# sIncerass/MVLPT

Measured on AMD Instinct MI355X. Metric: prompt-tuning images/sec (fwd+bwd), ViT-B/16 bs=256, 1/2/4/8 MI355X, higher is better.
Workload: dtype fp16; 1 GPU; BASELINE configs[1]: MVLPT coop head, ViT-B/16, 100 classes (caltech101 token table), n_ctx=16 n_vpt=0, text L=77, class token middle; text_positions_evaluated=77, step_pipelining=True, grad_precision=split_grad, layernorm_folding=both towers, residual_stream=packed fp16 + byte (image tower without prompts / backward), cu_partition=none (towers share every compute unit), per_gpu_batch=256, global_batch=256, parallelism=dp1, text_tower=replicated per GPU

## Files before the change

include/mvlpt_hip.h:

```cpp
#ifndef MVLPT_HIP_H
#define MVLPT_HIP_H
#include <stdint.h>
#ifdef __cplusplus
extern "C" {
#endif

typedef void* mvlpt_stream_t;

enum { MVLPT_DT_F32 = 0, MVLPT_DT_F16 = 1, MVLPT_DT_BF16 = 2 };
enum { MVLPT_LABEL_INT64 = 0, MVLPT_LABEL_PROB_F32 = 1 };
enum { MVLPT_ERR_ARG = -1, MVLPT_ERR_HIP = -2, MVLPT_ERR_STATE = -3, MVLPT_ERR_UNSUPPORTED = -4 };

typedef struct MvlptArch {
  int image_resolution, patch_size, vision_width, vision_layers, vision_heads;
  int context_length, text_width, text_layers, text_heads;
  int embed_dim;
  int compute_dtype;
} MvlptArch;

enum { MVLPT_PREC_FAST = 0, MVLPT_PREC_SPLIT_GRAD = 1, MVLPT_PREC_SPLIT_ALL = 2 };

int mvlpt_create(const MvlptArch* arch, void** handle);
int mvlpt_set_precision(void* handle, int mode);
int mvlpt_set_ln_fold(void* handle, int mode, int min_rows);
// ... 61 lines not shown
int mvlpt_op_attention32_bwd(int dtype, const void* qkv, const void* out, const void* dout, const float* lse, float* delta,
                             void* dqkv, int N, int L, int H, int causal, mvlpt_stream_t stream);
int mvlpt_op_pack_weight_mixed(int dtype, const float* w32, int rows, int cols, int transposed, void* out, int* w8_exp,
                               mvlpt_stream_t stream);
int mvlpt_op_gemm_mixed(int dtype, int epi, const void* A, const void* Bt, int ldb, int w8_exp, int M, int N, int K, const float* bias,
                        const void* aux, const float* resid, void* out, void* out2, mvlpt_stream_t stream);
int mvlpt_op_cast_mixed(int dtype, const float* in, void* out, int64_t rows, int d, mvlpt_stream_t stream);
int mvlpt_op_fold_vectors(int dtype, const void* W16, int ld, const float* gamma, const float* beta, const float* b, float* colsum,
                          float* bias2, int N, int K, mvlpt_stream_t stream);
int mvlpt_op_gemm_ln_producer(int dtype, const void* A, int a_split, const void* Bt, int ldb, int w8_exp, int M, int N, int K,
                              const float* bias, const float* resid, const float* gamma, int x16_split, float* out32, void* x16,
                              float* part, int ntp, int* nt, mvlpt_stream_t stream);
int mvlpt_op_gemm_folded(int dtype, int epi, const void* A16, int a_split, const void* Bt, int ldb, int w8_exp, int M, int N, int K,
                         const float* colsum, const float* bias2, const float* part, int ntp, int nt, void* out, void* out2,
                         mvlpt_stream_t stream);
int mvlpt_op_fold_weight(const void* W16, int ld, const float* gamma, void* Wg16, int ldg, float* colsum, int N, int K,
                         mvlpt_stream_t stream);
int mvlpt_op_respk_pack(const float* x, void* hi, uint8_t* lo, float* part, int ntp, int rows, int d, mvlpt_stream_t stream);
int mvlpt_op_assemble_packed(const float* patch_emb, const float* cls, const float* pos, const float* ln_g, const float* ln_b, void* hi,
                             uint8_t* lo, float* part, int ntp, int batch, int grid2, int d, mvlpt_stream_t stream);
int mvlpt_op_respk_unpack(const void* hi, const uint8_t* lo, int row_mul, float* out, int rows, int d, mvlpt_stream_t stream);
int mvlpt_op_gemm_residp(const void* A, const void* Bt, int ldb, int M, int N, int K, const float* bias, const void* hi_in,
                         const uint8_t* lo_in, void* hi_out, uint8_t* lo_out, float* part, int ntp, int* nt, mvlpt_stream_t stream);
int mvlpt_op_layernorm_fwd_mixed(int out_dtype, const float* x, const float* gamma, const float* beta, void* y, int rows, int d,
                                 mvlpt_stream_t stream);
int mvlpt_op_layernorm_bwd_mixed(int dtype, const void* dy, const float* x, const float* gamma, const float* resid, float* out32,
                                 void* out16, int rows, int d, mvlpt_stream_t stream);
int mvlpt_op_attention32_fwd_mixed(int dtype, const void* qkv, void* out, float* lse, int N, int L, int H, int causal, int q_rows,
                                   mvlpt_stream_t stream);
int mvlpt_op_attention32_bwd_mixed(int dtype, const void* qkv, const void* out, const void* dout, const float* lse, float* delta,
                                   void* dqkv, int N, int L, int H, int causal, mvlpt_stream_t stream);
int mvlpt_op_layernorm_fwd(int out_dtype, const float* x, const float* gamma, const float* beta, void* y, int rows, int d,
                           mvlpt_stream_t stream);
int mvlpt_op_layernorm_bwd(int dtype, const void* dy, const float* x, const float* gamma, const float* resid, float* out32,
                           void* out16, int rows, int d, mvlpt_stream_t stream);
int mvlpt_op_attention_fwd(int dtype, const void* qkv, void* out, float* lse, int N, int L, int H, int causal,
                           mvlpt_stream_t stream);
int mvlpt_op_attention_bwd(int dtype, const void* qkv, const void* out, const void* dout, const float* lse, float* delta,
                           void* dqkv, int N, int L, int H, int causal, mvlpt_stream_t stream);
int mvlpt_op_cast(int dtype, const float* in, void* out, int64_t n, mvlpt_stream_t stream);
int mvlpt_op_assemble_prompts_grouped(const float* prefix, const float* suffix, const float* ctx, int n_ctx, const int32_t* layout,
                                      const float* pos, float* x, int G, int C, int L, int d, mvlpt_stream_t stream);
int mvlpt_op_gather_ctx_grad_grouped(const float* dx, const int32_t* ctx_pos, int G, int C, int L, int d, int n_ctx, float* dctx,
                                     mvlpt_stream_t stream);
int mvlpt_op_assemble_prompts_ranged(const float* prefix, const float* suffix, const float* ctx, int n_ctx, const int32_t* layout,
                                     const float* pos, float* x, const int32_t* class_lo, const int32_t* class_hi, int G, int C, int L,
                                     int d, mvlpt_stream_t stream);
int mvlpt_op_gather_ctx_grad_ranged(const float* dx, const int32_t* ctx_pos, const int32_t* class_lo, const int32_t* class_hi, int G, int C,
                                    int L, int d, int n_ctx, float* dctx, mvlpt_stream_t stream);

int mvlpt_op_sgemm_bt(const float* A, const float* Bt, float* C, int M, int N, int K, const float* alpha_dev, mvlpt_stream_t stream);
int mvlpt_op_grad_scale(const float* v, int64_t n, float target, float* scale_dev, mvlpt_stream_t stream);
int mvlpt_op_reduce_prompt_rows(int dtype, float* dx32, void* dx16, int B, int L, int d, int row0, int n, float* out,
                                const float* scale_dev, int zero_after, int split16, const float* vmask, mvlpt_stream_t stream);
// ... 42 lines not shown
```

mvlpt_amd/_lib.py:

```python
from __future__ import annotations

import ctypes as C
import os

import torch

_HERE = os.path.dirname(os.path.abspath(__file__))
LIB_PATH = os.environ.get("MVLPT_HIP_LIB") or os.path.join(_HERE, "libmvlpt_hip.so")

DT_F32, DT_F16, DT_BF16 = 0, 1, 2
LABEL_INT64, LABEL_PROB_F32 = 0, 1
EPI_STORE16, EPI_GELU, EPI_RESID32, EPI_GELUBWD, EPI_STORE32, EPI_GELU_SPLIT, EPI_GELUBWD_SPLIT, EPI_STORE_SPLIT = 0, 1, 2, 3, 4, 5, 6, 7
GEMM_BT_128x128_R2, GEMM_BT_128x128_R4, GEMM_BT_256x128_R3, GEMM_BT_256x256_R2, GEMM_PHASED, GEMM_PC, GEMM_PCP = 1, 2, 3, 4, 5, 6, 7
PREC_FAST, PREC_SPLIT_GRAD, PREC_SPLIT_ALL = 0, 1, 2


class MvlptArch(C.Structure):
    _fields_ = [(n, C.c_int) for n in (
        "image_resolution", "patch_size", "vision_width", "vision_layers", "vision_heads",
        "context_length", "text_width", "text_layers", "text_heads", "embed_dim", "compute_dtype")]


class MvlptKernelStat(C.Structure):
    _fields_ = [("name", C.c_char * 32), ("launches", C.c_int64), ("ms", C.c_double),
# ... 53 lines not shown
    "mvlpt_op_gemm_ln_producer": (_i, [_i, _vp, _i, _vp, _i, _i, _i, _i, _i, _vp, _vp, _vp, _i, _vp, _vp, _vp, _i, C.POINTER(C.c_int), _vp]),
    "mvlpt_op_gemm_folded": (_i, [_i, _i, _vp, _i, _vp, _i, _i, _i, _i, _i, _vp, _vp, _vp, _i, _i, _vp, _vp, _vp]),
    "mvlpt_op_fold_weight": (_i, [_vp, _i, _vp, _vp, _i, _vp, _i, _i, _vp]),
    "mvlpt_op_respk_pack": (_i, [_vp, _vp, _vp, _vp, _i, _i, _i, _vp]),
    "mvlpt_op_assemble_packed": (_i, [_vp, _vp, _vp, _vp, _vp, _vp, _vp, _vp, _i, _i, _i, _i, _vp]),
    "mvlpt_op_respk_unpack": (_i, [_vp, _vp, _i, _vp, _i, _i, _vp]),
    "mvlpt_op_gemm_residp": (_i, [_vp, _vp, _i, _i, _i, _i, _vp, _vp, _vp, _vp, _vp, _vp, _i, C.POINTER(C.c_int), _vp]),
    "mvlpt_op_layernorm_fwd_mixed": (_i, [_i, _vp, _vp, _vp, _vp, _i, _i, _vp]),
    "mvlpt_op_layernorm_bwd_mixed": (_i, [_i, _vp, _vp, _vp, _vp, _vp, _vp, _i, _i, _vp]),
    "mvlpt_op_attention32_fwd_mixed": (_i, [_i, _vp, _vp, _vp, _i, _i, _i, _i, _i, _vp]),
    "mvlpt_op_attention32_bwd_mixed": (_i, [_i, _vp, _vp, _vp, _vp, _vp, _vp, _i, _i, _i, _i, _vp]),
    "mvlpt_op_layernorm_fwd": (_i, [_i, _vp, _vp, _vp, _vp, _i, _i, _vp]),
    "mvlpt_op_layernorm_bwd": (_i, [_i, _vp, _vp, _vp, _vp, _vp, _vp, _i, _i, _vp]),
    "mvlpt_op_attention_fwd": (_i, [_i, _vp, _vp, _vp, _i, _i, _i, _i, _vp]),
    "mvlpt_op_attention_bwd": (_i, [_i, _vp, _vp, _vp, _vp, _vp, _vp, _i, _i, _i, _i, _vp]),
    "mvlpt_op_cast": (_i, [_i, _vp, _vp, C.c_int64, _vp]),
    "mvlpt_op_assemble_prompts_grouped": (_i, [_vp, _vp, _vp, _i, _vp, _vp, _vp, _i, _i, _i, _i, _vp]),
    "mvlpt_op_gather_ctx_grad_grouped": (_i, [_vp, _vp, _i, _i, _i, _i, _i, _vp, _vp]),
    "mvlpt_op_assemble_prompts_ranged": (_i, [_vp, _vp, _vp, _i, _vp, _vp, _vp, _vp, _vp, _i, _i, _i, _i, _vp]),
    "mvlpt_op_gather_ctx_grad_ranged": (_i, [_vp, _vp, _vp, _vp, _i, _i, _i, _i, _i, _vp, _vp]),
    "mvlpt_op_sgemm_bt": (_i, [_vp, _vp, _vp, _i, _i, _i, _vp, _vp]),
    "mvlpt_op_grad_scale": (_i, [_vp, C.c_int64, _f, _vp, _vp]),
    "mvlpt_op_reduce_prompt_rows": (_i, [_i, _vp, _vp, _i, _i, _i, _i, _i, _vp, _vp, _i, _i, _vp, _vp]),
    "mvlpt_op_gather_ctx_grad": (_i, [_vp, _vp, _i, _i, _i, _i, _i, _vp, _vp, _vp]),
    "mvlpt_op_attention_bwd_cls": (_i, [_i, _vp, _vp, _vp, _vp, _vp, _i, _i, _i, _vp]),
    "mvlpt_op_copy_rows": (_i, [_vp, _vp, _vp, _i, _i, _i, _vp]),
    "mvlpt_op_overwrite_rows": (_i, [_vp, _i, _vp, _i, _i, _i, _vp, _vp]),
    "mvlpt_op_assemble_tokens": (_i, [_vp, _vp, _vp, _vp, _vp, _vp, _i, _vp, _vp, _i, _i, _i, _vp]),
    "mvlpt_op_assemble_prompts": (_i, [_vp, _vp, _vp, _i, _i, _vp, _vp, _vp, _vp, _vp, _vp, _i, _i, _i, _vp]),
    "mvlpt_preprocess": (_i, [_vp, _vp, C.c_int64, C.POINTER(MvlptImageDesc), _i, _i, _i, C.POINTER(_f), C.POINTER(_f), _vp, _i, _vp, _vp]),
# ... 30 lines not shown
```

mvlpt_amd/csrc/attention.hip:

```cpp
#include <hip/hip_ext.h>
#include "attn_common.h"

namespace mvlpt {

constexpr int ATT_MAX_NKT = 38;
int attn_max_len() { return ATT_MAX_NKT * 16; }

template <typename T, int NKT, bool CAUSAL>
__global__ __launch_bounds__(256) void attn_fwd_kernel(AttnArgs a) {
  extern __shared__ __attribute__((aligned(16))) char smem[];
  using v8 = typename Vec<T>::v8;
  using v4 = typename Vec<T>::v4;
  constexpr int LP = NKT * 16;
  constexpr int BLK = NKT < 16 ? NKT : 16;
  constexpr bool PRELOAD = NKT <= 16;
  char* sK = smem;
  char* sV = smem + LP * 128;
  const int L = a.L, H = a.H, d = H * 64;
  const int n = blockIdx.x / H, h = blockIdx.x % H;
  const size_t ld = (size_t)3 * d;
  const T* base = (const T*)a.qkv + (size_t)n * L * ld + h * 64;
  const int lane = threadIdx.x & 63, wave = __builtin_amdgcn_readfirstlane(threadIdx.x >> 6);
  const int fr = lane & 15, fg = lane >> 4;
  const int nqt = a.q_rows > 0 ? ((a.q_rows < L ? a.q_rows : L) + 15) >> 4 : (L + 15) >> 4;
// ... 465 lines not shown
        *(v4*)(gp + d + dt * 16) = wv;
      }
    }
  };
  if constexpr (PRELOAD) {
#pragma unroll
    for (int ki = 0; ki < MAXK; ++ki) {
      if (wave + 4 * ki >= nkt_all) break;
      process(wave + 4 * ki, pre[ki]);
    }
  } else {
    for (int kt = wave; kt < nkt_all; kt += 4) process(kt, load_kv(kt));
  }
}

template <typename T>
__device__ __forceinline__ float cls_dot16(const float* g16, const typename Vec<T>::v8& a0, const typename Vec<T>::v8& a1) {
  float s = 0.f;
#pragma unroll
  for (int e = 0; e < 8; ++e) { s = fmaf(g16[e], to_f32<T>(a0[e]), s); s = fmaf(g16[e + 8], to_f32<T>(a1[e]), s); }
  s += __shfl_xor(s, 1, 64); s += __shfl_xor(s, 2, 64);
  return s;
}
template <typename T>
__global__ __launch_bounds__(256) void attn_bwd_cls_kernel(const T* __restrict__ qkv, const T* __restrict__ o_cls,
                                                           const T* __restrict__ do_cls, const float* __restrict__ lse,
                                                           T* __restrict__ dqkv, int N, int L, int H) {
  using v8 = typename Vec<T>::v8;
  __shared__ float sq[64], sdo[64], red[4][64];
  const int n = blockIdx.x / H, h = blockIdx.x % H, d = H * 64, tid = threadIdx.x;
// ... 163 lines not shown
```

mvlpt_amd/csrc/engine.hip:

```cpp
#include <hip/hip_runtime.h>

#include <cmath>
#include <cstdio>
#include <algorithm>
#include <array>
#include <map>
#include <cstring>
#include <mutex>
#include <string>
#include <vector>

#include "../../include/mvlpt_hip.h"
#include "kernels.h"

using namespace mvlpt;


namespace {
struct StreamPart { hipStream_t s; int cus; };
std::mutex g_part_mu;
std::vector<StreamPart> g_parts;
int device_cus() {
  static int cus = 0;
  if (!cus) {
// ... 102 lines not shown
  int vpt_mask_layers = 0, vpt_mask_B = 0, vpt_mask_n = 0, vpt_mask_d = 0;
  const float* v_mask = nullptr;
  bool lo8 = true;
  std::string err;
  TowerW vis, txt;
  void* conv_w = nullptr; int Kp = 0; float* cls_emb = nullptr; float* vpos = nullptr; LNp ln_pre, ln_post;
  float *vproj = nullptr, *vproj_t = nullptr;
  float* tpos = nullptr; LNp ln_final; float *tproj = nullptr, *tproj_t = nullptr;
  std::vector<void*> owned;
  DevBuf vis_ws, txt_ws, head_ws, ce_ws, tmp, pp_ws;
  TowerState vs, ts;
  int vB = 0, v_nvpt = 0, v_ndeep = 0; float* cls32 = nullptr; float* dcls32 = nullptr;
  float* xc32 = nullptr; void *ac16 = nullptr, *hc16 = nullptr, *gc16 = nullptr;
  bool v_cls_last = false; float *xcm32 = nullptr, *xco32 = nullptr, *dxc32 = nullptr, *dhc32 = nullptr;
  void *uc16 = nullptr, *duc16 = nullptr, *dxc16 = nullptr, *dOc16 = nullptr;
  int tC = 0, tL = 0, t_nctx = 0, t_per_class = 0; int32_t* eot_rows = nullptr; int32_t* ctx_pos = nullptr;
  int t_groups = 0, t_gC = 0;
  bool t_ranged = false; const int32_t *t_rlo = nullptr, *t_rstart = nullptr;
  std::vector<int32_t> t_range_host, h_range_host;
  bool t_eot_last = false; float *txc32 = nullptr, *txm32 = nullptr, *txo32 = nullptr, *tdxc32 = nullptr, *tdhc32 = nullptr;
  void *tac16 = nullptr, *thc16 = nullptr, *tgc16 = nullptr, *tuc16 = nullptr, *tduc16 = nullptr, *tdxc16 = nullptr, *tdOc16 = nullptr;
  float* eot32 = nullptr; float* deot32 = nullptr;
  int hB = 0, hC = 0; float h_scale = 0.f; const int32_t *h_lo = nullptr, *h_hi = nullptr;
  bool h_grouped = false;
  bool h_ranged = false; int hS = 0; const int32_t *h_rlo = nullptr, *h_rstart = nullptr, *h_rgrp = nullptr;
  float *imn = nullptr, *txn = nullptr, *inorm = nullptr, *tnorm = nullptr;
  unsigned long long* dbg_ck = nullptr; int dbg_ck_n = 0; bool dbg_ck_on = false;
  bool prof_on = false, prof_all = false; std::vector<ProfRec> prof; std::vector<hipEvent_t> ev_pool; size_t ev_used = 0;
};

// ... 633 lines not shown
  Engine* E = (Engine*)h;
  if (!E || !image || !feat_out || B <= 0) return fail(E, MVLPT_ERR_ARG, "image_fwd: null/invalid argument");
  if (int rc = mvlpt_frozen_ready(h)) return rc;
  if ((n_vpt > 0) != (vpt != nullptr)) return fail(E, MVLPT_ERR_ARG, "image_fwd: vpt pointer and n_vpt disagree");
  if ((n_deep > 0) != (vpt_deep != nullptr) || (n_deep > 0 && n_vpt <= 0)) return fail(E, MVLPT_ERR_ARG, "image_fwd: deep prompts need vpt");
  hipStream_t s = (hipStream_t)stream;
  const MvlptArch& A = E->arch;
  const int G = A.image_resolution / A.patch_size, G2 = G * G, dv = A.vision_width, e = A.embed_dim;
  const int Lv = 1 + n_vpt + G2;
  if (Lv > attn_max_len()) return fail(E, MVLPT_ERR_UNSUPPORTED, "image_fwd: sequence length > 256 not supported yet");
  const bool save = save_for_bwd != 0;
  const bool exact = E->prec_mode == MVLPT_PREC_SPLIT_ALL || (E->prec_mode == MVLPT_PREC_SPLIT_GRAD && save);
  const size_t X = exact ? 2 : 1;
  const size_t npatch = (size_t)B * G2;
  size_t need = tower_bytes(E->vis, B, Lv, save, exact) + align256(npatch * E->Kp * 2) + align256(npatch * dv * 4) +
                7 * align256((size_t)B * dv * 4) + 4 * align256((size_t)B * dv * 2 * X) + 3 * align256((size_t)B * dv * 8 * X) + 4096;
  E->vs.valid = false;
  HIPCHK(E, E->vis_ws.reserve(need));
  Bump bp; bp.base = (char*)E->vis_ws.p; bp.cap = E->vis_ws.cap;
  void* patches = bp.take_bytes(npatch * E->Kp * 2);
  float* pe = bp.take<float>(npatch * dv);
  E->cls32 = bp.take<float>((size_t)B * dv);
  E->dcls32 = bp.take<float>((size_t)B * dv);
  E->xc32 = bp.take<float>((size_t)B * dv);
  E->ac16 = bp.take_bytes((size_t)B * dv * 2 * X); E->hc16 = bp.take_bytes((size_t)B * dv * 2 * X);
  E->gc16 = bp.take_bytes((size_t)B * dv * 4 * 2 * X);
  E->xcm32 = bp.take<float>((size_t)B * dv); E->xco32 = bp.take<float>((size_t)B * dv);
  E->dxc32 = bp.take<float>((size_t)B * dv); E->dhc32 = bp.take<float>((size_t)B * dv);
  E->dxc16 = bp.take_bytes((size_t)B * dv * 2 * X); E->dOc16 = bp.take_bytes((size_t)B * dv * 2 * X);
  E->uc16 = bp.take_bytes((size_t)B * dv * 4 * 2); E->duc16 = bp.take_bytes((size_t)B * dv * 4 * 2 * X);
  E->v_cls_last = false;
  carve_tower(bp, E->vis, E->vs, B, Lv, save, false, exact, split_kind(E));
  TowerState& st = E->vs;
  E->vB = B; E->v_nvpt = n_vpt; E->v_ndeep = n_deep;
  st.fold = E->fold_mode >= 1 && (size_t)B * Lv >= (size_t)E->fold_min_rows && dv >= 256;
  if (st.fold) if (int rc = prepare_fold(E, s)) return rc;

  const float* const masks = E->vpt_mask;
  const int mask_layers = E->vpt_mask_layers, mask_B = E->vpt_mask_B, mask_n = E->vpt_mask_n;
  E->vpt_mask = nullptr; E->vpt_mask_layers = 0; E->v_mask = nullptr;
  if (masks && (n_vpt <= 0 || mask_layers < 1 + n_deep || mask_B != B || mask_n != n_vpt))
    return fail(E, MVLPT_ERR_ARG, "image_fwd: the prompt dropout masks do not match this forward (layers >= 1 + n_deep, batch, n_vpt)");
  E->v_mask = masks;
  auto vmask = [&](int l) -> const float* { return masks ? masks + (size_t)l * B * n_vpt * dv : nullptr; };
  { ProfScope ps(E, s, PC_GLUE, 0, (double)npatch * E->Kp * 6.0);
// ... 44 lines not shown
    ln1_ready = produced;
  }
  if (cls_only_last) {
    const int l = E->vis.layers - 1;
    const Block& Bk = E->vis.blocks[l];
    const int T = B * Lv;
    float* xin = st.x[2 * l];
    float* xmid = save ? E->xcm32 : E->xc32;
    float* xout = save ? E->xco32 : E->xc32;
    E->v_cls_last = save;
    const int xs = st.xs;
    Fold fq;
    if (ln1_ready) fq = fold_consumer(st, 0, Bk.qkv);
    else HIPCHK(E, ln_fwd(E, E->dt, xin, nullptr, 1, Bk.ln1, st.h16, T, dv, s, xs));
    if (packed) fq.fold_colsum = Bk.qkv.fold_sg;
    HIPCHK(E, gemm(E, xs ? EPI_STORE_SPLIT : EPI_STORE16, packed ? xhi : st.h16, packed ? Bk.qkv.fwg() : Bk.qkv.fw(), T, 3 * dv, dv,
                   ln1_ready ? Bk.qkv.fold_b : Bk.qkv.b, nullptr, nullptr, st.qkv[l], nullptr, s, -1, xs, ln1_ready ? &fq : nullptr));
    dbg_ck(E, st.qkv[l], (size_t)T * 3 * dv * 2 * X, s);
    if (xs) {
      if (save) HIPCHK(E, launch_zero(st.attn[l], (size_t)T * dv * 4, s));
      if (int rc = attn32_fwd(E, st, l, 1, s)) return rc;
    } else {
      AttnArgs a{st.qkv[l], st.attn[l], save ? st.lse[l] : nullptr, st.N, st.L, st.H, 0, 1};
      ProfScope ps(E, s, PC_ATTN_FWD, 4.0 * st.L * 64.0 * st.N * st.H, (double)T * dv * 2.0 * 2.0);
      HIPCHK(E, launch_attn_fwd(E->dt, a, s));
    }
    { ProfScope ps(E, s, PC_GLUE, 0, (double)B * dv * 12.0);
      HIPCHK(E, launch_copy_rows_strided(st.attn[l], E->ac16, B, (size_t)Lv * dv * 2 * X, (size_t)dv * 2 * X, (int)(dv * 2 * X), s));
      if (packed) HIPCHK(E, launch_respk_unpack_rows(xhi, xlo, Lv, E->xc32, B, dv, s));
      else HIPCHK(E, launch_copy_rows_strided(xin, E->xc32, B, (size_t)Lv * dv * 4, (size_t)dv * 4, dv * 4, s)); }
    dbg_ck(E, E->ac16, (size_t)B * dv * 2 * X, s); dbg_ck(E, E->xc32, (size_t)B * dv * 4, s);
    HIPCHK(E, gemm(E, EPI_RESID32, E->ac16, Bk.o.fw(), B, dv, dv, Bk.o.b, nullptr, E->xc32, xmid, nullptr, s, -1, xs));
    HIPCHK(E, ln_fwd(E, E->dt, xmid, nullptr, 1, Bk.ln2, E->hc16, B, dv, s, xs));
    HIPCHK(E, gemm(E, xs ? EPI_GELU_SPLIT : EPI_GELU, E->hc16, Bk.fc.fw(), B, 4 * dv, dv, Bk.fc.b, nullptr, nullptr, E->gc16, save ? E->uc16 : nullptr, s, -1, xs));
    HIPCHK(E, gemm(E, EPI_RESID32, E->gc16, Bk.pr.fw(), B, dv, 4 * dv, Bk.pr.b, nullptr, xmid, xout, nullptr, s, -1, xs));
    HIPCHK(E, ln_fwd(E, DT_F32, xout, nullptr, 1, E->ln_post, E->cls32, B, dv, s));
  } else
  HIPCHK(E, ln_fwd(E, DT_F32, st.x[2 * E->vis.layers], nullptr, Lv, E->ln_post, E->cls32, B, dv, s));
  { ProfScope ps(E, s, PC_HEAD, 2.0 * B * e * dv, 4.0 * ((double)B * dv + (double)e * dv + (double)B * e));
    HIPCHK(E, launch_sgemm_bt(E->cls32, E->vproj_t, feat_out, B, e, dv, nullptr, s)); }
  return 0;
}

// ... 622 lines not shown
  OPCHK(launch_ln_fwd(out_dtype, a, (hipStream_t)stream));
  return 0;
}
int mvlpt_op_layernorm_bwd(int dtype, const void* dy, const float* x, const float* gamma, const float* resid, float* out32,
                           void* out16, int rows, int d, mvlpt_stream_t stream) {
  LnBwdArgs a{dy, dtype, x, nullptr, 1, gamma, resid, out32, out16, rows, d};
  OPCHK(launch_ln_bwd(dtype, a, (hipStream_t)stream));
  return 0;
}
int mvlpt_op_attention_fwd(int dtype, const void* qkv, void* out, float* lse, int N, int L, int H, int causal,
                           mvlpt_stream_t stream) {
  AttnArgs a{qkv, out, lse, N, L, H, causal};
  OPCHK(launch_attn_fwd(dtype, a, (hipStream_t)stream));
  return 0;
}
int mvlpt_op_attention_bwd(int dtype, const void* qkv, const void* out, const void* dout, const float* lse, float* delta,
                           void* dqkv, int N, int L, int H, int causal, mvlpt_stream_t stream) {
  AttnBwdArgs a{qkv, out, dout, lse, delta, dqkv, N, L, H, causal};
  OPCHK(launch_attn_bwd(dtype, a, (hipStream_t)stream));
  return 0;
}
int mvlpt_op_cast(int dtype, const float* in, void* out, int64_t n, mvlpt_stream_t stream) {
  OPCHK(launch_cast_f32_to16(dtype, in, out, (size_t)n, nullptr, (hipStream_t)stream));
  return 0;
}
int mvlpt_op_assemble_prompts_grouped(const float* prefix, const float* suffix, const float* ctx, int n_ctx, const int32_t* layout,
                                      const float* pos, float* x, int G, int C, int L, int d, mvlpt_stream_t stream) {
  if (!prefix || !suffix || !ctx || !layout || !pos || !x || G <= 0 || C <= 0 || L <= n_ctx + 1 || n_ctx <= 0 || d <= 0) {
    g_create_err = "op_assemble_prompts_grouped: null/invalid argument"; return MVLPT_ERR_ARG; }
  OPCHK(launch_assemble_prompts_grouped(prefix, suffix, ctx, n_ctx, layout, pos, x, G, C, L, d, (hipStream_t)stream));
// ... 203 lines not shown
```

mvlpt_amd/csrc/gemm.hip:

```cpp
#include <cstdlib>
#include <hip/hip_ext.h>
#include "kernels.h"
#include "gemm_epi.h"

namespace mvlpt {

#ifdef MVLPT_GEMM_TRACE
constexpr int TR_MAX = 2048;
#define MVLPT_TR(p) do { if (g.trace && blockIdx.x == 0 && lane == 0 && tr_n < TR_MAX) \
    g.trace[wave * TR_MAX + tr_n++] = ((long long)(p) << 56) | ((long long)__builtin_amdgcn_s_memtime() & 0xffffffffffffffLL); } while (0)
#else
#define MVLPT_TR(p) do { } while (0)
#endif

template <typename T, int EPI, int BM_, int BN_, int NW, int NS, bool MIXED>
__global__ __launch_bounds__(NW * 64, (NW == 2 || BM_ * BN_ / NW > 8192) ? 1 : 2) void gemm_bt_kernel(GemmArgs g) {
  extern __shared__ __attribute__((aligned(16))) char smem[];
  using v8 = typename Vec<T>::v8;
  constexpr int BN = BN_;
  constexpr int WCN = BN_ / 64, WCM = NW / WCN;
  constexpr int WMF = BM_ / WCM / 16;
  constexpr int A_BYTES = BM_ * BK * 2, B_BYTES = BN * BK * 2, STAGE = A_BYTES + B_BYTES;
  constexpr int A_IT = BM_ / 8 / NW, B_IT = BN / 8 / NW, LOADS = A_IT + B_IT;
  constexpr int ST_MIN_ = (WMF / 4) * ((epi_base(EPI) == EPI_STORE16 || epi_base(EPI) == EPI_GELU) ? 8 : 16);
// ... 941 lines not shown

static bool gemm_args_ok(int dtype, int epi, const GemmArgs& g, bool folded, bool dry) {
  if (dtype != DT_F16 && dtype != DT_BF16) return false;
  if (g.M <= 0 || g.N <= 0 || g.K <= 0 || (g.K % BK) != 0 || (g.N % 128) != 0 || g.a_split < 0 || g.a_split > 2) return false;
  if (g.a_split == 2 && (g.K % 128) != 0) return false;
  if (epi == EPI_RESIDP_LN && (dtype != DT_F16 || g.a_split)) return false;
  if (folded) {
    const bool can = epi == EPI_STORE16 || epi == EPI_GELU || epi == EPI_STORE_SPLIT || epi == EPI_GELU_SPLIT;
    const int nk = g.a_split == 2 ? g.K / BK + g.K / 128 : (g.a_split ? 2 : 1) * (g.K / BK);
    if (!can || g.fold_ntp <= 0 || g.fold_ntp > FOLD_MAX_NTP || (g.fold_ntp & 1) || nk < 4) return false;
  }
  if (dry) return true;
  if (g.a_split == 2 && g.ldb < g.K + g.K / 2) return false;
  if (g.ldb && (g.ldb < g.K || (g.ldb % 8) != 0)) return false;
  if (g.lda && (g.lda < (g.a_split ? 2 : 1) * g.K || (g.lda % 8) != 0)) return false;
  if (g.ldo && (g.ldo < 2 * g.N || (g.ldo % 8) != 0 || !(epi == EPI_GELU_SPLIT || epi == EPI_GELUBWD_SPLIT || epi == EPI_STORE_SPLIT))) return false;
  if ((epi == EPI_RESID32 || epi == EPI_RESID32_LN) && !g.resid) return false;
  if (epi == EPI_RESID32_LN && (!g.ln_gamma || !g.ln_x16 || !g.ln_part || g.ln_ntp <= 0 || (g.ln_ntp & 1))) return false;
  if (epi == EPI_RESIDP_LN && (!g.rp_hi_in || !g.rp_lo_in || !g.rp_lo_out || !g.ln_part || g.ln_ntp <= 0 || (g.ln_ntp & 1))) return false;
  if (folded && (!g.fold_colsum || !g.bias || g.fold_nt <= 0 || g.fold_nt > g.fold_ntp)) return false;
  if ((epi == EPI_GELUBWD || epi == EPI_GELUBWD_SPLIT) && !g.aux) return false;
  return true;
}

hipError_t gemm_route(int dtype, int epi, const GemmArgs& g, bool folded, hipStream_t s, GemmRoute* r) {
  if (!r || !gemm_args_ok(dtype, epi, g, folded, true)) return hipErrorInvalidValue;
  *r = GemmRoute{};
  const hipError_t e = dtype == DT_F16 ? launch_epi<f16>(g, epi, folded, s, (hipEvent_t)-1, nullptr, r)
                                       : launch_epi<bf16>(g, epi, folded, s, (hipEvent_t)-1, nullptr, r);
  if (e != hipSuccess) return e;
  switch (r->family) {
// ... 49 lines not shown
```

mvlpt_amd/csrc/gemm_epi.h:

```cpp
#pragma once
#include "kernels.h"

namespace mvlpt {

constexpr int BK = 64;

constexpr int EPI_SCRATCH_PER_WAVE = 4608;

template <int RS>
struct LinearRows {
  char* base;
  __device__ __forceinline__ char* operator()(int r) const { return base + r * RS; }
};
template <int RS>
struct SlabRows {
  static constexpr int RPS = 1024 / RS;
  char* slot; int wave; int a_bytes;
  __device__ __forceinline__ char* operator()(int r) const {
    const int sl = r / RPS, k = r - sl * RPS;
    const int off = sl < 4 ? (sl * 8 + wave) * 1024 : a_bytes + ((sl - 4) * 8 + wave) * 1024;
    return slot + off + k * RS;
  }
};

// ... 148 lines not shown
            for (int j = 0; j < 4; ++j) {
              const f32x4 v = acc[i][j] + bv[j];
              v4 w;
#pragma unroll
              for (int e = 0; e < 4; ++e) w[e] = from_f32<T>((EPI == EPI_GELU && which == 0) ? quick_gelu(v[e]) : v[e]);
              *(v4*)(rows16(ii * 16 + fr) + (j * 16 + fg * 4) * 2) = w;
            }
          }
        }
        asm volatile("s_waitcnt lgkmcnt(0)" ::: "memory");
        {
          const int c = lane & 7, r0 = lane >> 3;
          v8 w[4];
#pragma unroll
          for (int it = 0; it < 4; ++it) w[it] = *(const v8*)(rows16(it * 8 + r0) + c * 16);
          T* const o0 = outp + (size_t)(mbase + half * 32 + r0) * N + nbase + c * 8;
          if (mbase + half * 32 + 32 <= M) {
#pragma unroll
            for (int it = 0; it < 4; ++it) __builtin_nontemporal_store(w[it], (v8*)(o0 + (size_t)it * 8 * N));
          } else {
#pragma unroll
            for (int it = 0; it < 4; ++it)
              if (mbase + half * 32 + it * 8 + r0 < M) __builtin_nontemporal_store(w[it], (v8*)(o0 + (size_t)it * 8 * N));
          }
        }
        asm volatile("s_waitcnt lgkmcnt(0)" ::: "memory");
      }
    }
  } else if constexpr (EPI == EPI_RESIDP_LN) {
    static_assert(__is_same(T, f16), "the packed residual stream is an fp16 format");
    int c = lane & 7, rq = lane >> 3;
    asm volatile("" : "+v"(c), "+v"(rq));
    v8 uv[4][2];
    typedef unsigned u32x2 __attribute__((ext_vector_type(2)));
    u32x2 lw[4][2];
#pragma unroll
    for (int i = 0; i < 4; ++i)
#pragma unroll
// ... 136 lines not shown
```

mvlpt_amd/csrc/kernels.h:

```cpp
#pragma once
#include "common.h"

namespace mvlpt {

int stream_cus(hipStream_t s);

enum GemmEpi {
  EPI_STORE16 = 0,
  EPI_GELU = 1,
  EPI_RESID32 = 2,
  EPI_GELUBWD = 3,
  EPI_STORE32 = 4,
  EPI_GELU_SPLIT = 5,
  EPI_GELUBWD_SPLIT = 6,
  EPI_STORE_SPLIT = 7,
  EPI_RESID32_LN = 8,
  EPI_STORE16_FOLD = 9, EPI_GELU_FOLD = 10, EPI_STORE_SPLIT_FOLD = 11, EPI_GELU_SPLIT_FOLD = 12,
  EPI_RESIDP_LN = 13,
};
constexpr int epi_base(int epi) {
  return epi == EPI_STORE16_FOLD ? EPI_STORE16 : epi == EPI_GELU_FOLD ? EPI_GELU : epi == EPI_STORE_SPLIT_FOLD ? EPI_STORE_SPLIT
         : epi == EPI_GELU_SPLIT_FOLD ? EPI_GELU_SPLIT : epi;
}
constexpr bool epi_folds(int epi) { return epi >= EPI_STORE16_FOLD && epi <= EPI_GELU_SPLIT_FOLD; }
// ... 69 lines not shown

struct AttnArgs {
  const void* qkv; void* out ; float* lse ;
  int N, L, H; int causal;
  int q_rows = 0;
  int flags = 0;
};
hipError_t launch_attn_fwd(int dtype, const AttnArgs& a, hipStream_t s, hipEvent_t ea = nullptr, hipEvent_t eb = nullptr);
struct AttnBwdArgs {
  const void* qkv; const void* out; const void* dout; const float* lse;
  float* delta ; void* dqkv ;
  int N, L, H; int causal;
};
hipError_t launch_attn_bwd(int dtype, const AttnBwdArgs& a, hipStream_t s);
int attn_max_len();
hipError_t launch_attn_bwd_cls(int dtype, const void* qkv, const void* o_cls, const void* do_cls, const float* lse, void* dqkv,
                               int N, int L, int H, hipStream_t s);
hipError_t launch_attn_fwd_stream(int dtype, const AttnArgs& a, hipStream_t s);
hipError_t launch_attn_bwd_stream(int dtype, const AttnBwdArgs& a, hipStream_t s);

struct Attn32Args {
  const void* qkv_split;
  void* out_split;
  float* lse;
  int N, L, H; int causal;
  int q_rows = 0;
  int out_lo8 = 0;
#ifdef MVLPT_ATTN_TRACE
  long long* trace = nullptr;
#endif
// ... 89 lines not shown
```

mvlpt_amd/engine.py:

```python
from __future__ import annotations

import ctypes as C
from typing import Dict, List, Optional, Tuple

import torch

from . import _lib
from ._lib import DT_BF16, DT_F16, DT_F32, lib
from .weights import ClipArch, arch_from_state_dict

_TORCH2DT = {torch.float32: DT_F32, torch.float16: DT_F16, torch.bfloat16: DT_BF16}
_DT2TORCH = {DT_F16: torch.float16, DT_BF16: torch.bfloat16, DT_F32: torch.float32}


def _ptr(t: Optional[torch.Tensor]):
    return None if t is None else C.c_void_p(t.data_ptr())


def _stream() -> C.c_void_p:
    return C.c_void_p(torch.cuda.current_stream().cuda_stream)


def _on_device(fn):
    import functools
# ... 698 lines not shown
    out32 = torch.empty(rows, d, device=x.device, dtype=torch.float32)
    out16 = torch.empty(rows, d, device=x.device, dtype=dy.dtype) if want16 else None
    _lib.check(lib.mvlpt_op_layernorm_bwd(_TORCH2DT[dy.dtype], _ptr(dy), _ptr(x), _ptr(gamma), _ptr(resid), _ptr(out32),
                                          _ptr(out16), rows, d, _stream()), None, "op_layernorm_bwd")
    return out32, out16


def op_attention_fwd(qkv, N, L, H, causal, want_lse=True):
    out = torch.empty(N * L, H * 64, device=qkv.device, dtype=qkv.dtype)
    lse = torch.empty(N * H * L, device=qkv.device, dtype=torch.float32) if want_lse else None
    _lib.check(lib.mvlpt_op_attention_fwd(_TORCH2DT[qkv.dtype], _ptr(qkv), _ptr(out), _ptr(lse), N, L, H, int(causal), _stream()),
               None, "op_attention_fwd")
    return out, lse


def op_attention_bwd(qkv, out, dout, lse, N, L, H, causal):
    dqkv = torch.empty_like(qkv)
    delta = torch.empty(N * H * L, device=qkv.device, dtype=torch.float32)
    _lib.check(lib.mvlpt_op_attention_bwd(_TORCH2DT[qkv.dtype], _ptr(qkv), _ptr(out), _ptr(dout), _ptr(lse), _ptr(delta),
                                          _ptr(dqkv), N, L, H, int(causal), _stream()), None, "op_attention_bwd")
    return dqkv


def op_fold_vectors(W16: torch.Tensor, K: int, gamma, beta, b):
    N, ld = W16.shape
    cs = torch.empty(N, device=W16.device, dtype=torch.float32)
    b2 = torch.empty(N, device=W16.device, dtype=torch.float32)
    _lib.check(lib.mvlpt_op_fold_vectors(_TORCH2DT[W16.dtype], _ptr(W16), ld, _ptr(gamma), _ptr(beta), _ptr(b), _ptr(cs), _ptr(b2), N, K,
                                         _stream()), None, "op_fold_vectors")
    return cs, b2
# ... 77 lines not shown
```

Before: 19100 images/sec.

## Compute only CLS query row in last vision layer QKV and attention

In the last vision layer, where only the CLS token output is needed, the QKV projection is split in two. K and V are computed for all tokens, while Q is computed only for the B CLS rows, using a strided row-copy of the fold partials. A new single-query attention kernel writes CLS outputs directly into the compact buffer, which removes full-sequence Q projection and full attention for that layer along with one row-copy. It adds a small partial-copy kernel, an extra GEMM launch, and strided-output support in the STORE16 epilogue.

```diff
diff --git a/include/mvlpt_hip.h b/include/mvlpt_hip.h
--- a/include/mvlpt_hip.h
+++ b/include/mvlpt_hip.h
@@ -99,6 +99,9 @@
 int mvlpt_op_gemm_folded(int dtype, int epi, const void* A16, int a_split, const void* Bt, int ldb, int w8_exp, int M, int N, int K,
                          const float* colsum, const float* bias2, const float* part, int ntp, int nt, void* out, void* out2,
                          mvlpt_stream_t stream);
+int mvlpt_op_gemm_folded_ex(int dtype, int epi, const void* A16, int a_split, const void* Bt, int ldb, int w8_exp, int M, int N, int K,
+                            const float* colsum, const float* bias2, const float* part, int ntp, int nt, void* out, void* out2, int lda,
+                            int ldo, mvlpt_stream_t stream);
 int mvlpt_op_fold_weight(const void* W16, int ld, const float* gamma, void* Wg16, int ldg, float* colsum, int N, int K,
                          mvlpt_stream_t stream);
 int mvlpt_op_respk_pack(const float* x, void* hi, uint8_t* lo, float* part, int ntp, int rows, int d, mvlpt_stream_t stream);
@@ -123,6 +126,8 @@
                            mvlpt_stream_t stream);
 int mvlpt_op_attention_bwd(int dtype, const void* qkv, const void* out, const void* dout, const float* lse, float* delta,
                            void* dqkv, int N, int L, int H, int causal, mvlpt_stream_t stream);
+int mvlpt_op_attention_fwd_cls(int dtype, const void* qkv, void* out, int64_t out_ld, float* lse, int N, int L, int H, int generic,
+                               mvlpt_stream_t stream);
 int mvlpt_op_cast(int dtype, const float* in, void* out, int64_t n, mvlpt_stream_t stream);
 int mvlpt_op_assemble_prompts_grouped(const float* prefix, const float* suffix, const float* ctx, int n_ctx, const int32_t* layout,
                                       const float* pos, float* x, int G, int C, int L, int d, mvlpt_stream_t stream);
diff --git a/mvlpt_amd/_lib.py b/mvlpt_amd/_lib.py
--- a/mvlpt_amd/_lib.py
+++ b/mvlpt_amd/_lib.py
@@ -91,6 +91,8 @@
     "mvlpt_op_layernorm_bwd": (_i, [_i, _vp, _vp, _vp, _vp, _vp, _vp, _i, _i, _vp]),
     "mvlpt_op_attention_fwd": (_i, [_i, _vp, _vp, _vp, _i, _i, _i, _i, _vp]),
     "mvlpt_op_attention_bwd": (_i, [_i, _vp, _vp, _vp, _vp, _vp, _vp, _i, _i, _i, _i, _vp]),
+    "mvlpt_op_attention_fwd_cls": (_i, [_i, _vp, _vp, C.c_int64, _vp, _i, _i, _i, _i, _vp]),
+    "mvlpt_op_gemm_folded_ex": (_i, [_i, _i, _vp, _i, _vp, _i, _i, _i, _i, _i, _vp, _vp, _vp, _i, _i, _vp, _vp, _i, _i, _vp]),
     "mvlpt_op_cast": (_i, [_i, _vp, _vp, C.c_int64, _vp]),
     "mvlpt_op_assemble_prompts_grouped": (_i, [_vp, _vp, _vp, _i, _vp, _vp, _vp, _i, _i, _i, _i, _vp]),
     "mvlpt_op_gather_ctx_grad_grouped": (_i, [_vp, _vp, _i, _i, _i, _i, _i, _vp, _vp]),
diff --git a/mvlpt_amd/csrc/attention.hip b/mvlpt_amd/csrc/attention.hip
--- a/mvlpt_amd/csrc/attention.hip
+++ b/mvlpt_amd/csrc/attention.hip
@@ -503,6 +503,89 @@
   }
 }
 
+__device__ __forceinline__ float row8_sum_dpp(float v) {
+  v += __builtin_bit_cast(float, __builtin_amdgcn_update_dpp(0, __builtin_bit_cast(int, v), 0xB1, 0xF, 0xF, true));
+  v += __builtin_bit_cast(float, __builtin_amdgcn_update_dpp(0, __builtin_bit_cast(int, v), 0x4E, 0xF, 0xF, true));
+  v += __builtin_bit_cast(float, __builtin_amdgcn_update_dpp(0, __builtin_bit_cast(int, v), 0x141, 0xF, 0xF, true));
+  return v;
+}
+template <typename T>
+__global__ __launch_bounds__(256) void attn_fwd_cls_kernel(const T* __restrict__ qkv, T* __restrict__ out, size_t out_ld,
+                                                           float* __restrict__ lse, int N, int L, int H) {
+  using v8 = typename Vec<T>::v8;
+  const int lane = threadIdx.x & 63;
+  const int item = blockIdx.x * 4 + (threadIdx.x >> 6);
+  if (item >= N * H) return;
+  const int n = item / H, h = item - n * H, d = H * 64;
+  const size_t ld = (size_t)3 * d;
+  const int g = lane >> 3, c8 = (lane & 7) * 8;
+  const T* base = qkv + (size_t)n * L * ld + h * 64 + c8;
+  constexpr float SC = 0.125f * 1.4426950408889634f;
+  float q[8], acc[8];
+  {
+    const v8 qv = *(const v8*)base;
+#pragma unroll
+    for (int e = 0; e < 8; ++e) { q[e] = to_f32<T>(qv[e]) * SC; acc[e] = 0.f; }
+  }
+  float m = -INFINITY, l = 0.f;
+  constexpr int UB = 4;
+  for (int j0 = 0; j0 < L; j0 += 8 * UB) {
+    v8 kv[UB], vv[UB];
+#pragma unroll
+    for (int u = 0; u < UB; ++u) {
+      const int j = j0 + u * 8 + g;
+      const T* kp = base + (size_t)(j < L ? j : L - 1) * ld + d;
+      kv[u] = __builtin_nontemporal_load((const v8*)kp);
+      vv[u] = __builtin_nontemporal_load((const v8*)(kp + d));
+    }
+#pragma unroll
+    for (int u = 0; u < UB; ++u) {
+      const int j = j0 + u * 8 + g;
+      float sc = 0.f;
+#pragma unroll
+      for (int e = 0; e < 8; ++e) sc = fmaf(q[e], to_f32<T>(kv[u][e]), sc);
+      sc = row8_sum_dpp(sc);
+      if (j < L) {
+        const float mn = fmaxf(m, sc);
+        const float alpha = __builtin_amdgcn_exp2f(m - mn);
+        const float p = __builtin_amdgcn_exp2f(sc - mn);
+        m = mn;
+        l = fmaf(l, alpha, p);
+#pragma unroll
+        for (int e = 0; e < 8; ++e) acc[e] = fmaf(acc[e], alpha, p * to_f32<T>(vv[u][e]));
+      }
+    }
+  }
+  float mx = m;
+  mx = fmaxf(mx, __shfl_xor(mx, 8, 64)); mx = fmaxf(mx, __shfl_xor(mx, 16, 64)); mx = fmaxf(mx, __shfl_xor(mx, 32, 64));
+  const float w = __builtin_amdgcn_exp2f(m - mx);
+  l *= w;
+  l += __shfl_xor(l, 8, 64); l += __shfl_xor(l, 16, 64); l += __shfl_xor(l, 32, 64);
+  const float inv = 1.0f / l;
+  v8 o;
+#pragma unroll
+  for (int e = 0; e < 8; ++e) {
+    float a = acc[e] * w;
+    a += __shfl_xor(a, 8, 64); a += __shfl_xor(a, 16, 64); a += __shfl_xor(a, 32, 64);
+    o[e] = from_f32<T>(a * inv);
+  }
+  if (g == 0) {
+    *(v8*)(out + (size_t)n * out_ld + h * 64 + c8) = o;
+    if (lse && lane == 0) lse[((size_t)n * H + h) * L] = (mx + log2f(l)) * 0.6931471805599453f;
+  }
+}
+hipError_t launch_attn_fwd_cls(int dtype, const void* qkv, void* out, size_t out_ld, float* lse, int N, int L, int H, hipStream_t s,
+                               hipEvent_t ea, hipEvent_t eb) {
+  if (N <= 0 || L <= 0 || H <= 0 || out_ld < (size_t)H * 64 || (out_ld % 8) != 0) return hipErrorInvalidValue;
+  const int blocks = (int)(((long)N * H + 3) / 4);
+  if (dtype == DT_F16)
+    hipExtLaunchKernelGGL(attn_fwd_cls_kernel<f16>, dim3(blocks), dim3(256), 0, s, ea, eb, 0, (const f16*)qkv, (f16*)out, out_ld, lse, N, L, H);
+  else if (dtype == DT_BF16)
+    hipExtLaunchKernelGGL(attn_fwd_cls_kernel<bf16>, dim3(blocks), dim3(256), 0, s, ea, eb, 0, (const bf16*)qkv, (bf16*)out, out_ld, lse, N, L, H);
+  else return hipErrorInvalidValue;
+  return hipGetLastError();
+}
+
 template <typename T>
 __device__ __forceinline__ float cls_dot16(const float* g16, const typename Vec<T>::v8& a0, const typename Vec<T>::v8& a1) {
   float s = 0.f;
diff --git a/mvlpt_amd/csrc/engine.hip b/mvlpt_amd/csrc/engine.hip
--- a/mvlpt_amd/csrc/engine.hip
+++ b/mvlpt_amd/csrc/engine.hip
@@ -140,6 +140,7 @@
   float* xc32 = nullptr; void *ac16 = nullptr, *hc16 = nullptr, *gc16 = nullptr;
   bool v_cls_last = false; float *xcm32 = nullptr, *xco32 = nullptr, *dxc32 = nullptr, *dhc32 = nullptr;
   void *uc16 = nullptr, *duc16 = nullptr, *dxc16 = nullptr, *dOc16 = nullptr;
+  float* cpart = nullptr;
   int tC = 0, tL = 0, t_nctx = 0, t_per_class = 0; int32_t* eot_rows = nullptr; int32_t* ctx_pos = nullptr;
   int t_groups = 0, t_gC = 0;
   bool t_ranged = false; const int32_t *t_rlo = nullptr, *t_rstart = nullptr;
@@ -803,7 +804,8 @@
   const size_t X = exact ? 2 : 1;
   const size_t npatch = (size_t)B * G2;
   size_t need = tower_bytes(E->vis, B, Lv, save, exact) + align256(npatch * E->Kp * 2) + align256(npatch * dv * 4) +
-                7 * align256((size_t)B * dv * 4) + 4 * align256((size_t)B * dv * 2 * X) + 3 * align256((size_t)B * dv * 8 * X) + 4096;
+                7 * align256((size_t)B * dv * 4) + 4 * align256((size_t)B * dv * 2 * X) + 3 * align256((size_t)B * dv * 8 * X) +
+                align256((size_t)B * FOLD_NTP * 8) + 4096;
   E->vs.valid = false;
   HIPCHK(E, E->vis_ws.reserve(need));
   Bump bp; bp.base = (char*)E->vis_ws.p; bp.cap = E->vis_ws.cap;
@@ -818,6 +820,7 @@
   E->dxc32 = bp.take<float>((size_t)B * dv); E->dhc32 = bp.take<float>((size_t)B * dv);
   E->dxc16 = bp.take_bytes((size_t)B * dv * 2 * X); E->dOc16 = bp.take_bytes((size_t)B * dv * 2 * X);
   E->uc16 = bp.take_bytes((size_t)B * dv * 4 * 2); E->duc16 = bp.take_bytes((size_t)B * dv * 4 * 2 * X);
+  E->cpart = bp.take<float>((size_t)B * FOLD_NTP * 2);
   E->v_cls_last = false;
   carve_tower(bp, E->vis, E->vs, B, Lv, save, false, exact, split_kind(E));
   TowerState& st = E->vs;
@@ -892,19 +895,38 @@
     if (ln1_ready) fq = fold_consumer(st, 0, Bk.qkv);
     else HIPCHK(E, ln_fwd(E, E->dt, xin, nullptr, 1, Bk.ln1, st.h16, T, dv, s, xs));
     if (packed) fq.fold_colsum = Bk.qkv.fold_sg;
-    HIPCHK(E, gemm(E, xs ? EPI_STORE_SPLIT : EPI_STORE16, packed ? xhi : st.h16, packed ? Bk.qkv.fwg() : Bk.qkv.fw(), T, 3 * dv, dv,
-                   ln1_ready ? Bk.qkv.fold_b : Bk.qkv.b, nullptr, nullptr, st.qkv[l], nullptr, s, -1, xs, ln1_ready ? &fq : nullptr));
+    const void* const qa = packed ? xhi : st.h16;
+    const WRef qw = packed ? Bk.qkv.fwg() : Bk.qkv.fw();
+    const float* const qb = ln1_ready ? Bk.qkv.fold_b : Bk.qkv.b;
+    if (xs) {
+      HIPCHK(E, gemm(E, EPI_STORE_SPLIT, qa, qw, T, 3 * dv, dv, qb, nullptr, nullptr, st.qkv[l], nullptr, s, -1, xs, ln1_ready ? &fq : nullptr));
+    } else {
+      if (E->dbg_ck_on) HIPCHK(E, launch_zero(st.qkv[l], (size_t)T * 3 * dv * 2, s));
+      const int ldw = qw.ld ? qw.ld : dv;
+      const WRef wkv{(const char*)qw.p + (size_t)dv * ldw * 2, qw.ld, qw.e8};
+      Fold fkv = fq, fqc = fq;
+      if (ln1_ready) {
+        fkv.fold_colsum = fq.fold_colsum + dv;
+        ProfScope ps(E, s, PC_GLUE, 0, (double)B * fq.fold_ntp * 16.0);
+        HIPCHK(E, launch_copy_rows_strided(fq.fold_part, E->cpart, B, (size_t)Lv * fq.fold_ntp * 8, (size_t)fq.fold_ntp * 8, fq.fold_ntp * 8, s));
+        fqc.fold_part = E->cpart;
+      }
+      HIPCHK(E, gemm(E, EPI_STORE16, qa, wkv, T, 2 * dv, dv, qb + dv, nullptr, nullptr, (char*)st.qkv[l] + (size_t)dv * 2, nullptr, s, -1, 0,
+                     ln1_ready ? &fkv : nullptr, 0, 3 * dv));
+      HIPCHK(E, gemm(E, EPI_STORE16, qa, qw, B, dv, dv, qb, nullptr, nullptr, st.qkv[l], nullptr, s, -1, 0, ln1_ready ? &fqc : nullptr,
+                     Lv * dv, Lv * 3 * dv));
+    }
     dbg_ck(E, st.qkv[l], (size_t)T * 3 * dv * 2 * X, s);
     if (xs) {
       if (save) HIPCHK(E, launch_zero(st.attn[l], (size_t)T * dv * 4, s));
       if (int rc = attn32_fwd(E, st, l, 1, s)) return rc;
+      ProfScope ps(E, s, PC_GLUE, 0, (double)B * dv * 8.0);
+      HIPCHK(E, launch_copy_rows_strided(st.attn[l], E->ac16, B, (size_t)Lv * dv * 2 * X, (size_t)dv * 2 * X, (int)(dv * 2 * X), s));
     } else {
-      AttnArgs a{st.qkv[l], st.attn[l], save ? st.lse[l] : nullptr, st.N, st.L, st.H, 0, 1};
       ProfScope ps(E, s, PC_ATTN_FWD, 4.0 * st.L * 64.0 * st.N * st.H, (double)T * dv * 2.0 * 2.0);
-      HIPCHK(E, launch_attn_fwd(E->dt, a, s));
+      HIPCHK(E, launch_attn_fwd_cls(E->dt, st.qkv[l], E->ac16, (size_t)dv, save ? st.lse[l] : nullptr, st.N, st.L, st.H, s));
     }
-    { ProfScope ps(E, s, PC_GLUE, 0, (double)B * dv * 12.0);
-      HIPCHK(E, launch_copy_rows_strided(st.attn[l], E->ac16, B, (size_t)Lv * dv * 2 * X, (size_t)dv * 2 * X, (int)(dv * 2 * X), s));
+    { ProfScope ps(E, s, PC_GLUE, 0, (double)B * dv * 8.0);
       if (packed) HIPCHK(E, launch_respk_unpack_rows(xhi, xlo, Lv, E->xc32, B, dv, s));
       else HIPCHK(E, launch_copy_rows_strided(xin, E->xc32, B, (size_t)Lv * dv * 4, (size_t)dv * 4, dv * 4, s)); }
     dbg_ck(E, E->ac16, (size_t)B * dv * 2 * X, s); dbg_ck(E, E->xc32, (size_t)B * dv * 4, s);
@@ -1557,6 +1579,28 @@
   OPCHK(launch_attn_fwd(dtype, a, (hipStream_t)stream));
   return 0;
 }
+int mvlpt_op_attention_fwd_cls(int dtype, const void* qkv, void* out, int64_t out_ld, float* lse, int N, int L, int H, int generic,
+                               mvlpt_stream_t stream) {
+  if (!qkv || !out) { g_create_err = "op_attention_fwd_cls: null argument"; return MVLPT_ERR_ARG; }
+  if (generic) {
+    if (out_ld != (int64_t)L * H * 64) { g_create_err = "op_attention_fwd_cls: the tiled kernel writes row 0 of [N*L, d]"; return MVLPT_ERR_ARG; }
+    AttnArgs a{qkv, out, lse, N, L, H, 0, 1};
+    OPCHK(launch_attn_fwd(dtype, a, (hipStream_t)stream));
+    return 0;
+  }
+  OPCHK(launch_attn_fwd_cls(dtype, qkv, out, (size_t)out_ld, lse, N, L, H, (hipStream_t)stream));
+  return 0;
+}
+int mvlpt_op_gemm_folded_ex(int dtype, int epi, const void* A16, int a_split, const void* Bt, int ldb, int w8_exp, int M, int N, int K,
+                            const float* colsum, const float* bias2, const float* part, int ntp, int nt, void* out, void* out2, int lda,
+                            int ldo, mvlpt_stream_t stream) {
+  GemmArgs g{A16, Bt, M, N, K, bias2, nullptr, nullptr, out, out2};
+  g.a_split = a_split; g.ldb = ldb; g.w8_exp = w8_exp; g.lda = lda; g.ldo = ldo;
+  g.out_lo8 = (a_split == 2 && epi == EPI_GELU_SPLIT) ? 1 : 0;
+  g.fold_part = part; g.fold_colsum = colsum; g.fold_ntp = ntp; g.fold_nt = nt;
+  OPCHK(launch_gemm(dtype, epi, g, (hipStream_t)stream));
+  return 0;
+}
 int mvlpt_op_attention_bwd(int dtype, const void* qkv, const void* out, const void* dout, const float* lse, float* delta,
                            void* dqkv, int N, int L, int H, int causal, mvlpt_stream_t stream) {
   AttnBwdArgs a{qkv, out, dout, lse, delta, dqkv, N, L, H, causal};
diff --git a/mvlpt_amd/csrc/gemm.hip b/mvlpt_amd/csrc/gemm.hip
--- a/mvlpt_amd/csrc/gemm.hip
+++ b/mvlpt_amd/csrc/gemm.hip
@@ -979,7 +979,10 @@
   if (g.a_split == 2 && g.ldb < g.K + g.K / 2) return false;
   if (g.ldb && (g.ldb < g.K || (g.ldb % 8) != 0)) return false;
   if (g.lda && (g.lda < (g.a_split ? 2 : 1) * g.K || (g.lda % 8) != 0)) return false;
-  if (g.ldo && (g.ldo < 2 * g.N || (g.ldo % 8) != 0 || !(epi == EPI_GELU_SPLIT || epi == EPI_GELUBWD_SPLIT || epi == EPI_STORE_SPLIT))) return false;
+  if (g.ldo) {
+    const bool pair = epi == EPI_GELU_SPLIT || epi == EPI_GELUBWD_SPLIT || epi == EPI_STORE_SPLIT;
+    if ((g.ldo % 8) != 0 || !(pair || epi == EPI_STORE16) || g.ldo < (pair ? 2 : 1) * g.N) return false;
+  }
   if ((epi == EPI_RESID32 || epi == EPI_RESID32_LN) && !g.resid) return false;
   if (epi == EPI_RESID32_LN && (!g.ln_gamma || !g.ln_x16 || !g.ln_part || g.ln_ntp <= 0 || (g.ln_ntp & 1))) return false;
   if (epi == EPI_RESIDP_LN && (!g.rp_hi_in || !g.rp_lo_in || !g.rp_lo_out || !g.ln_part || g.ln_ntp <= 0 || (g.ln_ntp & 1))) return false;
diff --git a/mvlpt_amd/csrc/gemm_epi.h b/mvlpt_amd/csrc/gemm_epi.h
--- a/mvlpt_amd/csrc/gemm_epi.h
+++ b/mvlpt_amd/csrc/gemm_epi.h
@@ -186,14 +186,15 @@
           v8 w[4];
 #pragma unroll
           for (int it = 0; it < 4; ++it) w[it] = *(const v8*)(rows16(it * 8 + r0) + c * 16);
-          T* const o0 = outp + (size_t)(mbase + half * 32 + r0) * N + nbase + c * 8;
+          const size_t ldo = (EPI == EPI_STORE16 && g.ldo) ? (size_t)g.ldo : (size_t)N;
+          T* const o0 = outp + (size_t)(mbase + half * 32 + r0) * ldo + nbase + c * 8;
           if (mbase + half * 32 + 32 <= M) {
 #pragma unroll
-            for (int it = 0; it < 4; ++it) __builtin_nontemporal_store(w[it], (v8*)(o0 + (size_t)it * 8 * N));
+            for (int it = 0; it < 4; ++it) __builtin_nontemporal_store(w[it], (v8*)(o0 + (size_t)it * 8 * ldo));
           } else {
 #pragma unroll
             for (int it = 0; it < 4; ++it)
-              if (mbase + half * 32 + it * 8 + r0 < M) __builtin_nontemporal_store(w[it], (v8*)(o0 + (size_t)it * 8 * N));
+              if (mbase + half * 32 + it * 8 + r0 < M) __builtin_nontemporal_store(w[it], (v8*)(o0 + (size_t)it * 8 * ldo));
           }
         }
         asm volatile("s_waitcnt lgkmcnt(0)" ::: "memory");
diff --git a/mvlpt_amd/csrc/kernels.h b/mvlpt_amd/csrc/kernels.h
--- a/mvlpt_amd/csrc/kernels.h
+++ b/mvlpt_amd/csrc/kernels.h
@@ -107,6 +107,8 @@
 };
 hipError_t launch_attn_bwd(int dtype, const AttnBwdArgs& a, hipStream_t s);
 int attn_max_len();
+hipError_t launch_attn_fwd_cls(int dtype, const void* qkv, void* out, size_t out_ld, float* lse, int N, int L, int H, hipStream_t s,
+                               hipEvent_t ea = nullptr, hipEvent_t eb = nullptr);
 hipError_t launch_attn_bwd_cls(int dtype, const void* qkv, const void* o_cls, const void* do_cls, const float* lse, void* dqkv,
                                int N, int L, int H, hipStream_t s);
 hipError_t launch_attn_fwd_stream(int dtype, const AttnArgs& a, hipStream_t s);
diff --git a/mvlpt_amd/engine.py b/mvlpt_amd/engine.py
--- a/mvlpt_amd/engine.py
+++ b/mvlpt_amd/engine.py
@@ -736,6 +736,24 @@
     return out, lse
 
 
+def op_attention_fwd_cls(qkv, N, L, H, generic=False, want_lse=True):
+    d = H * 64
+    lse = torch.zeros(N * H * L, device=qkv.device, dtype=torch.float32) if want_lse else None
+    out = torch.zeros(N * L if generic else N, d, device=qkv.device, dtype=qkv.dtype)
+    _lib.check(lib.mvlpt_op_attention_fwd_cls(_TORCH2DT[qkv.dtype], _ptr(qkv), _ptr(out), L * d if generic else d, _ptr(lse), N, L, H,
+                                              int(generic), _stream()), None, "op_attention_fwd_cls")
+    if generic:
+        out = out.view(N, L, d)[:, 0].contiguous()
+    return out, (lse.view(N, H, L)[:, :, 0].contiguous() if want_lse else None)
+
+
+def op_gemm_folded_ex(x16, Bt, colsum, bias2, part, nt, M, N, K, out, epi=_lib.EPI_STORE16, a_split=0, ldb=0, w8_exp=0, lda=0, ldo=0):
+    _lib.check(lib.mvlpt_op_gemm_folded_ex(_TORCH2DT[x16.dtype], epi, _ptr(x16), a_split, _ptr(Bt), ldb, w8_exp, M, N, K, _ptr(colsum),
+                                           _ptr(bias2), _ptr(part), part.shape[-2], nt, _ptr(out), None, lda, ldo, _stream()), None,
+               "op_gemm_folded_ex")
+    return out
+
+
 def op_attention_bwd(qkv, out, dout, lse, N, L, H, causal):
     dqkv = torch.empty_like(qkv)
     delta = torch.empty(N * H * L, device=qkv.device, dtype=torch.float32)
```

After: 19220 images/sec, median of 6. About the same (+0.6%).
